# Alexander-H-Liu/End-to-end-ASR-Pytorch

Hardware: AMD Instinct MI355X
Metric: audio frames/sec training (LAS+CTC, LibriSpeech 80-mel) (higher is better)
Workload: dtype f32; 1 GPU; cfg3: {"B": 32, "T": 1600, "D": 80, "V": 5000, "L": 64}; global_batch=32, parallelism=dp1

## Files before the change

end-to-end-asr-pytorch_amd/csrc/speller.hip:

```cpp
#include "common.h"
#include "knobs.h"
#include <cstdlib>

namespace {

__device__ __forceinline__ float tanh_fast(float x) {
    const float e = __expf(2.f * x);
    return 1.f - __fdividef(2.f, e + 1.f);
}
__device__ __forceinline__ float sigmoid_fast(float x) { return __fdividef(1.f, 1.f + __expf(-x)); }

unsigned long long *g_sp_dbg = nullptr;
int g_sp_dbg_slots = 0;
inline unsigned long long *sp_slot(int step, int kid) {
    const long i = (long)step * 16 + kid;
    return (g_sp_dbg && i < g_sp_dbg_slots) ? g_sp_dbg + i * 16 : nullptr;
}
#define SP_STAMP(ph)                                                                                     \
    do {                                                                                                 \
        if (p.stamps && threadIdx.x == 0) {                                                              \
            if (blockIdx.x == 0 && blockIdx.y == 0) p.stamps[ph] = __builtin_readcyclecounter();         \
            else if (blockIdx.x == gridDim.x - 1 && blockIdx.y == gridDim.y - 1 && ((ph) == 0 || (ph) == 9)) \
                p.stamps[(ph) == 0 ? 12 : 13] = __builtin_readcyclecounter();                            \
        }                                                                                                \
// ... 33 lines not shown
};

template <int VEC>
__device__ __forceinline__ void load8(const float *row, int k, int klen, bool valid, float (&v)[8]) {
    if (VEC && valid && k + 8 <= klen) {
        const f32x4 a = *reinterpret_cast<const f32x4 *>(row + k);
        const f32x4 b = *reinterpret_cast<const f32x4 *>(row + k + 4);
        v[0] = a[0]; v[1] = a[1]; v[2] = a[2]; v[3] = a[3];
        v[4] = b[0]; v[5] = b[1]; v[6] = b[2]; v[7] = b[3];
        return;
    }
#pragma unroll
    for (int j = 0; j < 8; ++j) v[j] = (valid && k + j < klen) ? row[k + j] : 0.f;
}

template <int MT, int EPI, int VEC>
__global__ __launch_bounds__(SK_THREADS) void skinny_kernel(SkArgs p) {
    __shared__ float red[SK_WAVES][MT][4][64];
    const int tid = threadIdx.x, lane = tid & 63;
    const int wave = __builtin_amdgcn_readfirstlane(tid >> 6);
    const int slot = lane & 15, g = lane >> 4;
    SP_STAMP(0);
    int r;
    bool rvalid;
    if (EPI == EPI_LSTM_FWD) {
        const int u = blockIdx.x * 4 + (slot >> 2);
        r = (slot & 3) * p.H + u;
        rvalid = u < p.H;
    } else {
        r = blockIdx.x * 16 + slot;
        rvalid = r < p.R;
    }
    f32x4 acc[MT][2];
#pragma unroll
    for (int mt = 0; mt < MT; ++mt) acc[mt][0] = acc[mt][1] = f32x4{0.f, 0.f, 0.f, 0.f};

    float e_in[EPI == EPI_LSTM_BWD ? 36 : 13];
    const bool e_thr = tid < MT * 64;
    const int e_m = (tid >> 6) * 16 + (lane & 15);
    if (e_thr && e_m < p.M) {
        if (EPI == EPI_STORE || EPI == EPI_TANH_BIAS) {
#pragma unroll
            for (int q = 0; q < 4; ++q) {
                const int rr = blockIdx.x * 16 + (lane >> 4) * 4 + q;
                e_in[q] = (rr < p.R && p.bias) ? p.bias[rr] : 0.f;
            }
        } else if (EPI == EPI_LSTM_FWD) {
            const int u = blockIdx.x * 4 + (lane >> 4), H = p.H;
            if (u < H) {
#pragma unroll
                for (int q = 0; q < 4; ++q) {
                    const long col = (long)q * H + u;
                    e_in[q] = p.pre ? p.pre[(long)e_m * 4 * H + col] : 0.f;
                    e_in[4 + q] = p.b0 ? p.b0[col] : 0.f;
                    e_in[8 + q] = p.b1 ? p.b1[col] : 0.f;
                }
                e_in[12] = p.c_prev[(long)e_m * H + u];
            }
        } else {
            const int H = p.H;
#pragma unroll
            for (int q = 0; q < 4; ++q) {
                const int j = blockIdx.x * 16 + (lane >> 4) * 4 + q;
                if (j >= H) continue;
                const float *gr = p.dG + (long)e_m * 4 * H + j;
                e_in[q * 9 + 0] = p.add0 ? p.add0[(long)e_m * p.ld0 + j] : 0.f;
                e_in[q * 9 + 1] = p.add1 ? p.add1[(long)e_m * p.ld1 + j] : 0.f;
                e_in[q * 9 + 2] = gr[0];
                e_in[q * 9 + 3] = gr[H];
                e_in[q * 9 + 4] = gr[2 * (long)H];
                e_in[q * 9 + 5] = gr[3 * (long)H];
                e_in[q * 9 + 6] = p.bc_new[(long)e_m * H + j];
                e_in[q * 9 + 7] = p.dc_valid ? p.dc[(long)e_m * H + j] : 0.f;
                e_in[q * 9 + 8] = p.bc_prev[(long)e_m * H + j];
            }
        }
    }

// ... 18 lines not shown
        const unsigned long long wp0 = sg64(p.seg[0].w), wp1 = sg64(p.seg[1].w), wp2 = sg64(p.seg[2].w);
        const unsigned long long xp0 = sg64(p.seg[0].x), xp1 = sg64(p.seg[1].x), xp2 = sg64(p.seg[2].x);
        const unsigned wb0 = sg(p.seg[0].wbytes), wb1 = sg(has1 ? p.seg[1].wbytes : 0u), wb2 = sg(has2 ? p.seg[2].wbytes : 0u);
        const unsigned xb0 = sg(p.seg[0].xbytes), xb1 = sg(has1 ? p.seg[1].xbytes : 0u), xb2 = sg(has2 ? p.seg[2].xbytes : 0u);
        const unsigned ldw0 = sg((unsigned)p.seg[0].ldw * 4u), ldw1 = sg((unsigned)p.seg[1].ldw * 4u), ldw2 = sg((unsigned)p.seg[2].ldw * 4u);
        const unsigned ldx0 = sg((unsigned)p.seg[0].ldx * 4u), ldx1 = sg((unsigned)p.seg[1].ldx * 4u), ldx2 = sg((unsigned)p.seg[2].ldx * 4u);
        const unsigned kl0 = sg((unsigned)p.seg[0].klen * 4u), kl1 = sg(has1 ? (unsigned)p.seg[1].klen * 4u : 0u),
                       kl2 = sg(has2 ? (unsigned)p.seg[2].klen * 4u : 0u);
        const int Mrows = (int)sg((unsigned)p.M);
        unsigned wrow[2];
        bool wok[2];
#pragma unroll
        for (int h = 0; h < 2; ++h) {
            const int sl = lrow + 8 * h;
            if (EPI == EPI_LSTM_FWD) {
                const int u = blockIdx.x * 4 + (sl >> 2);
                wrow[h] = (unsigned)((sl & 3) * p.H + u);
                wok[h] = u < p.H;
            } else {
                wrow[h] = (unsigned)(blockIdx.x * 16 + sl);
                wok[h] = (int)wrow[h] < p.R;
            }
        }
#define SK_ISSUE(i_, gw_, gx_)                                                                          \
    do {                                                                                                \
        const int c_ = wave + (i_) * SK_WAVES;                \
        const bool s1_ = c_ >= n0, s2_ = c_ >= n0 + n1;                                                 \
        const int base_ = s2_ ? n0 + n1 : (s1_ ? n0 : 0);                                               \
        const __amdgpu_buffer_rsrc_t rw_ = __builtin_amdgcn_make_buffer_rsrc(                           \
            reinterpret_cast<void *>(s2_ ? wp2 : (s1_ ? wp1 : wp0)), 0, (int)(s2_ ? wb2 : (s1_ ? wb1 : wb0)), 0x00020000); \
        const __amdgpu_buffer_rsrc_t rx_ = __builtin_amdgcn_make_buffer_rsrc(                           \
            reinterpret_cast<void *>(s2_ ? xp2 : (s1_ ? xp1 : xp0)), 0, (int)(s2_ ? xb2 : (s1_ ? xb1 : xb0)), 0x00020000); \
        const unsigned ldw_ = s2_ ? ldw2 : (s1_ ? ldw1 : ldw0), ldx_ = s2_ ? ldx2 : (s1_ ? ldx1 : ldx0); \
        const unsigned kl_ = s2_ ? kl2 : (s1_ ? kl1 : kl0);                                             \
        const unsigned kb_ = (unsigned)(c_ - base_) * (SK_CH * 4u) + (unsigned)lk * 4u;                 \
// ... 27 lines not shown
        };
        auto mfmas = [&acc](const f32x4 (&fw)[2], const f32x4 (&fx)[MT][2]) __attribute__((always_inline)) {
#pragma unroll
            for (int hh = 0; hh < 2; ++hh)
#pragma unroll
                for (int j = 0; j < 4; ++j)
#pragma unroll
                    for (int mt = 0; mt < MT; ++mt)
                        acc[mt][j & 1] = __builtin_amdgcn_mfma_f32_16x16x4f32(fw[hh][j], fx[mt][hh][j], acc[mt][j & 1], 0, 0, 0);
        };
        if (mych > 0) {
            u32x4 gw[NB][2], gx[NB][NX];
            f32x4 fw[2][2], fx[2][MT][2];
#pragma unroll
            for (int j = 0; j < NB; ++j) SK_ISSUE(j, gw[j], gx[j]);
            SP_STAMP(1);
            stage(gw[0], gx[0], fw[0], fx[0]);
            SP_STAMP(2);
            SK_ISSUE(NB, gw[0], gx[0]);
#define SK_STEP(u)                                                                                      \
    if (i0 + (u) >= mych) break;                                                                        \
    stage(gw[((u) + 1) % NB], gx[((u) + 1) % NB], fw[((u) + 1) & 1], fx[((u) + 1) & 1]);                \
    SK_ISSUE(i0 + (u) + 1 + NB, gw[((u) + 1) % NB], gx[((u) + 1) % NB]);                                \
    __builtin_amdgcn_sched_barrier(0);                                                                  \
    mfmas(fw[(u) & 1], fx[(u) & 1]);                                                                    \
    __builtin_amdgcn_sched_barrier(0);
            for (int i0 = 0; i0 < mych; i0 += NB) {
                SK_STEP(0)
                SK_STEP(1)
                if (NB > 2) {
                    SK_STEP(2)
                    SK_STEP(3)
                }
// ... 22 lines not shown
#pragma unroll
                for (int mt = 0; mt < MT; ++mt)
                    acc[mt][j & 1] = __builtin_amdgcn_mfma_f32_16x16x4f32(w0[j], x0[mt][j], acc[mt][j & 1], 0, 0, 0);
#pragma unroll
            for (int j = 0; j < 8; ++j)
#pragma unroll
                for (int mt = 0; mt < MT; ++mt)
                    acc[mt][j & 1] = __builtin_amdgcn_mfma_f32_16x16x4f32(w1[j], x1[mt][j], acc[mt][j & 1], 0, 0, 0);
        }
    }
    }
#pragma unroll
    for (int mt = 0; mt < MT; ++mt)
#pragma unroll
        for (int v = 0; v < 4; ++v) red[wave][mt][v][lane] = acc[mt][0][v] + acc[mt][1][v];
    SP_STAMP(3);
    __syncthreads();
    SP_STAMP(4);
    if (tid >= MT * 64) return;
    const int mt = tid >> 6;
    float v[4];
#pragma unroll
    for (int q = 0; q < 4; ++q) {
        float s = 0.f;
#pragma unroll
        for (int w = 0; w < SK_WAVES; ++w) s += red[w][mt][q][lane];
        v[q] = s;
    }
    const int m = mt * 16 + (lane & 15);
    if (m >= p.M) return;
    if (EPI == EPI_STORE || EPI == EPI_TANH_BIAS) {
#pragma unroll
        for (int q = 0; q < 4; ++q) {
            const int rr = blockIdx.x * 16 + (lane >> 4) * 4 + q;
            if (rr < p.R) {
                float y = v[q] + e_in[q];
                if (EPI == EPI_TANH_BIAS) y = tanh_fast(y);
                p.out[(long)m * p.ldo + rr] = y;
            }
        }
    } else if (EPI == EPI_LSTM_FWD) {
        const int u = blockIdx.x * 4 + (lane >> 4);
        if (u >= p.H) return;
        const int H = p.H;
        float a[4];
#pragma unroll
        for (int q = 0; q < 4; ++q) {
            const long col = (long)q * H + u;
            (void)col;
            a[q] = v[q] + e_in[q] + e_in[4 + q] + e_in[8 + q];
        }
        float hn;
        if (p.gru) {
            const float gr_ = sigmoid_fast(a[0]), gz = sigmoid_fast(a[1]), gn = tanh_fast(a[2] + gr_ * a[3]);
            hn = (1.f - gz) * gn + gz * e_in[12];
            if (p.gates) {
                float *gr = p.gates + (long)m * 4 * H + u;
// ... 4 lines not shown
                        go = sigmoid_fast(a[3]);
            const float cn = gf * e_in[12] + gi * gg;
            hn = go * tanh_fast(cn);
            if (p.gates) {
                float *gr = p.gates + (long)m * 4 * H + u;
                gr[0] = gi; gr[H] = gf; gr[2 * (long)H] = gg; gr[3 * (long)H] = go;
            }
            p.c_new[(long)m * H + u] = cn;
        }
        p.h_new[(long)m * H + u] = hn;
        if (p.h_bm) p.h_bm[(long)m * p.h_bm_ld + u] = hn;
    } else {
        const int H = p.H;
#pragma unroll
        for (int q = 0; q < 4; ++q) {
            const int j = blockIdx.x * 16 + (lane >> 4) * 4 + q;
            if (j >= H) continue;
            float *gr = p.dG + (long)m * 4 * H + j;
            if (p.gru) {
                const float dh = v[q] + e_in[q * 9 + 0] + e_in[q * 9 + 1] + e_in[q * 9 + 7];
                const float r_ = e_in[q * 9 + 2], z_ = e_in[q * 9 + 3], n_ = e_in[q * 9 + 4], nh = e_in[q * 9 + 5];
                const float dnp = dh * (1.f - z_) * (1.f - n_ * n_);
                gr[0] = dnp * nh * r_ * (1.f - r_);
                gr[H] = dh * (e_in[q * 9 + 8] - n_) * z_ * (1.f - z_);
                gr[2 * (long)H] = dnp;
                gr[3 * (long)H] = dnp * r_;
                p.dc[(long)m * H + j] = dh * z_;
                continue;
            }
            const float dh = v[q] + e_in[q * 9 + 0] + e_in[q * 9 + 1];
            const float gi = e_in[q * 9 + 2], gf = e_in[q * 9 + 3], gg = e_in[q * 9 + 4], go = e_in[q * 9 + 5];
            const float tc = tanh_fast(e_in[q * 9 + 6]);
            const float dct = dh * go * (1.f - tc * tc) + e_in[q * 9 + 7];
            gr[0] = dct * gg * gi * (1.f - gi);
            gr[H] = dct * e_in[q * 9 + 8] * gf * (1.f - gf);
            gr[2 * (long)H] = dct * gi * (1.f - gg * gg);
            gr[3 * (long)H] = dh * tc * go * (1.f - go);
            p.dc[(long)m * H + j] = dct * gf;
        }
    }
    SP_STAMP(9);
}

inline bool al16(const void *q) { return (reinterpret_cast<uintptr_t>(q) & 15) == 0; }

template <int EPI>
int launch_skinny(const SkArgs &a, hipStream_t s) {
    if (a.M <= 0) return ASRK_OK;
    bool vec = true;
    for (int i = 0; i < a.nseg; ++i)
        vec = vec && al16(a.seg[i].x) && al16(a.seg[i].w) && a.seg[i].ldx % 4 == 0 && a.seg[i].ldw % 4 == 0 &&
              a.seg[i].klen % 4 == 0;
    const int blocks = (EPI == EPI_LSTM_FWD) ? asrk_div_up(a.H, 4) : asrk_div_up(a.R, 16);
    if (blocks <= 0) return ASRK_OK;
    for (int m0 = 0; m0 < a.M; m0 += 64) {
        SkArgs p = a;
        p.M = a.M - m0 < 64 ? a.M - m0 : 64;
        for (int i = 0; i < p.nseg; ++i) p.seg[i].x += (long)m0 * p.seg[i].ldx;
        bool small = true;
        const long wrows = (EPI == EPI_LSTM_FWD) ? 4L * p.H : (long)p.R;
        for (int i = 0; i < p.nseg; ++i) {
            const long wb = ((wrows - 1) * p.seg[i].ldw + p.seg[i].klen) * 4L;
            const long xb = ((long)(p.M - 1) * p.seg[i].ldx + p.seg[i].klen) * 4L;
            small = small && wb < (1L << 31) && xb < (1L << 31);
            p.seg[i].wbytes = (unsigned)wb;
            p.seg[i].xbytes = (unsigned)xb;
        }
        for (int i = p.nseg; i < 3; ++i) p.seg[i] = SkSeg{nullptr, nullptr, 0, 0, 0, 0u, 0u};
        if (p.out) p.out += (long)m0 * p.ldo;
        const long H4 = 4L * p.H, H1 = p.H;
        if (p.pre) p.pre += m0 * H4;
        if (p.c_prev) p.c_prev += m0 * H1;
        if (p.c_new) p.c_new += m0 * H1;
        if (p.h_new) p.h_new += m0 * H1;
        if (p.gates) p.gates += m0 * H4;
        if (p.h_bm) p.h_bm += (long)m0 * p.h_bm_ld;
        if (p.add0) p.add0 += (long)m0 * p.ld0;
        if (p.add1) p.add1 += (long)m0 * p.ld1;
        if (p.dG) p.dG += m0 * H4;
        if (p.bc_prev) p.bc_prev += m0 * H1;
        if (p.bc_new) p.bc_new += m0 * H1;
        if (p.dc) p.dc += m0 * H1;
        const int mt = p.M <= 16 ? 1 : (p.M <= 32 ? 2 : 4);
#define SK_LAUNCH_V(MT_, V_)                                                                        \
    do {                                                                                            \
        static AsrkLdsLatch latch_;                                                                 \
        const size_t lds = (size_t)SK_WAVES * (16 + MT_ * 16) * 36 * sizeof(float);                 \
        hipError_t e_ = asrk_max_lds_once(latch_, reinterpret_cast<const void *>(&skinny_kernel<MT_, EPI, V_>), (int)lds); \
        if (e_ != hipSuccess) return (int)e_;                                                       \
        hipLaunchKernelGGL((skinny_kernel<MT_, EPI, V_>), dim3(blocks), dim3(SK_THREADS), lds, s, p); \
    } while (0)
#define SK_LAUNCH(MT_)                                                                              \
    do {                                                                                            \
        if (vec && small) SK_LAUNCH_V(MT_, 2);                                                      \
        else hipLaunchKernelGGL((skinny_kernel<MT_, EPI, 0>), dim3(blocks), dim3(SK_THREADS), 0, s, p); \
    } while (0)
        if (mt == 1) SK_LAUNCH(1);
        else if (mt == 2) SK_LAUNCH(2);
        else SK_LAUNCH(4);
#undef SK_LAUNCH
#undef SK_LAUNCH_V
    }
// ... 876 lines not shown
#pragma unroll
        for (int w = 0; w < 8; ++w) acc += s_dq[w][a];
        p.dq_part[((long)r * TC + chunk) * A + a] = acc;
    }
}

struct CbArgs {
    const float *dconv, *prev, *Wc, *dq_part, *q;
    float *dprev, *dWc_part, *dq_pre;
    long prev_ld;
    int Te, K, ks, TC, A, nT, want_dprev;
    unsigned long long *stamps;
    int dq_only;
};

__global__ __launch_bounds__(256) void conv_bwd_kernel(CbArgs p) {
    extern __shared__ float sm[];
    const int b = blockIdx.x, y = p.dq_only ? p.nT + p.K : blockIdx.y, tid = threadIdx.x;
    const int Te = p.Te, K = p.K, ks = p.ks, KW = 2 * ks + 1;
    SP_STAMP(0);
    if (y < p.nT) {
        if (!p.want_dprev) return;
        const int s0 = y * 64, span = 64 + 2 * ks;
        float *sd = sm, *part = sm + K * span;
        float *s_w = part + 256;
        for (int i = tid; i < span * K; i += 256) {
            const int o = i / K, k = i - o * K;
            const int t = s0 + o - ks;
            sd[k * span + o] = (t >= 0 && t < Te) ? p.dconv[((long)b * Te + t) * K + k] : 0.f;
        }
        for (int i = tid; i < K * KW; i += 256) s_w[i] = p.Wc[i];
        __syncthreads();
        const int sl = tid & 63, w = __builtin_amdgcn_readfirstlane(tid >> 6);
        float acc = 0.f;
        for (int k = w; k < K; k += 4) {
            const float *wr = s_w + k * KW;
            const float *col = sd + k * span + sl + 2 * ks;
            for (int j = 0; j < KW; ++j) acc += col[-j] * wr[j];
        }
        part[w * 64 + sl] = acc;
        __syncthreads();
        if (tid < 64 && s0 + tid < Te)
            p.dprev[(long)b * Te + s0 + tid] = (part[tid] + part[64 + tid]) + (part[128 + tid] + part[192 + tid]);
        SP_STAMP(9);
    } else if (y < p.nT + K) {
        const int k = y - p.nT;
        float *s_dc = sm, *s_pv = sm + Te;
        float old[4];
#pragma unroll
        for (int r = 0; r < 4; ++r) {
            const int j = tid + 256 * r;
            old[r] = j < KW ? p.dWc_part[((long)b * K + k) * KW + j] : 0.f;
        }
        for (int t = tid; t < Te; t += 256) s_dc[t] = p.dconv[((long)b * Te + t) * K + k];
        for (int i = tid; i < Te + 2 * ks; i += 256) {
            const int t = i - ks;
            s_pv[i] = (t >= 0 && t < Te) ? p.prev[(long)b * p.prev_ld + t] : 0.f;
        }
        __syncthreads();
#pragma unroll
        for (int r = 0; r < 4; ++r) {
            const int j = tid + 256 * r;
            if (j < KW) {
                const float *pv = s_pv + j;
                float acc = 0.f;
                for (int t = 0; t < Te; ++t) acc += s_dc[t] * pv[t];
                p.dWc_part[((long)b * K + k) * KW + j] = old[r] + acc;
            }
        }
        for (int j = tid + 1024; j < KW; j += 256) {
            const float *pv = s_pv + j;
            float acc = 0.f;
            for (int t = 0; t < Te; ++t) acc += s_dc[t] * pv[t];
            p.dWc_part[((long)b * K + k) * KW + j] += acc;
        }
    } else {
        for (int a = tid; a < p.A; a += 256) {
            float acc = 0.f;
            for (int c = 0; c < p.TC; ++c) acc += p.dq_part[((long)b * p.TC + c) * p.A + a];
            const float qv = p.q[(long)b * p.A + a];
            p.dq_pre[(long)b * p.A + a] = acc * (1.f - qv * qv);
        }
        SP_STAMP(9);
    }
}

constexpr int DV_LC = 64;
__global__ __launch_bounds__(256) void dvalue_kernel(const float *__restrict__ attn, long attn_ld,
                                                     long attn_step, const float *__restrict__ dxh,
                                                     long step_ld, long row_ld, float *__restrict__ dvalue,
                                                     int L, int Te, int Dv) {
    extern __shared__ float s_at[];
    const int b = blockIdx.x, d = blockIdx.y * 256 + threadIdx.x;
    for (int l0 = 0; l0 < L; l0 += DV_LC) {
        const int nl = min(DV_LC, L - l0);
        __syncthreads();
        for (int i = threadIdx.x; i < nl * Te; i += 256) {
            const int l = i / Te, t = i - l * Te;
// ... 1 lines not shown
        }
        for (int i = nl * Te + threadIdx.x; i < DV_LC * Te; i += 256) s_at[i] = 0.f;
        __syncthreads();
        if (d < Dv) {
            float g[DV_LC];
#pragma unroll
            for (int l = 0; l < DV_LC; ++l)
                g[l] = l < nl ? dxh[(long)(l0 + l) * step_ld + (long)b * row_ld + d] : 0.f;
            float *out = dvalue + (long)b * Te * Dv + d;
            for (int t = 0; t < Te; ++t) {
                float acc = 0.f;
#pragma unroll
                for (int l = 0; l < DV_LC; ++l) acc += s_at[l * Te + t] * g[l];
                if (l0 == 0) out[(long)t * Dv] = acc;
                else out[(long)t * Dv] += acc;
            }
        }
    }
}

__global__ __launch_bounds__(256) void joint_score_kernel(const float *__restrict__ att,
                                                          const int64_t *__restrict__ cand,
                                                          const float *__restrict__ psi,
                                                          const float *__restrict__ prev_ctc,
                                                          const float *__restrict__ lm, float *__restrict__ out,
                                                          int V, int C, float wa, float w_ctc, float w_lm,
                                                          float logzero) {
    const int r = blockIdx.x;
    const float *a = att + (long)r * V;
    const float *l = lm ? lm + (long)r * V : nullptr;
// ... 132 lines not shown
inline bool upper_ok(const asrk_speller_t &d, bool fwd) {
    for (int l = 1; l < n_layers(d); ++l)
        if (!d.Wu_ih[l - 1] || !d.Wu_hh[l - 1] || !d.hu[l - 1] || !d.cu[l - 1] || !d.gu[l - 1] ||
            (fwd && (!d.bu_ih[l - 1] || !d.bu_hh[l - 1])))
            return false;
    return true;
}

template <typename T>
int set_lds(T kernel, size_t bytes) {
    ASRK_HIP(hipFuncSetAttribute(reinterpret_cast<const void *>(kernel),
                                 hipFuncAttributeMaxDynamicSharedMemorySize, (int)bytes));
    return ASRK_OK;
}

}

extern "C" void asrk_prof_launches_(int id, int64_t n);

extern "C" int asrk_transpose_ld_f32(const float *in, int64_t ldi, float *out, int64_t ldo, int rows,
                                     int cols, void *stream) {
    if (rows < 0 || cols < 0 || ldi < cols || ldo < rows) return ASRK_EINVAL;
    if (rows == 0 || cols == 0) return ASRK_OK;
    if (!in || !out) return ASRK_EINVAL;
    hipLaunchKernelGGL(transpose_ld_kernel, dim3(asrk_div_up(cols, 32), asrk_div_up(rows, 32)), dim3(256), 0,
                       (hipStream_t)stream, in, (long)ldi, out, (long)ldo, rows, cols);
    ASRK_LAUNCH_CHECK();
    return ASRK_OK;
}

extern "C" int asrk_speller_dvalue_f32(const float *attn, int64_t attn_ld, int64_t attn_step, const float *dxh,
                                       int64_t step_ld, int64_t row_ld, float *dvalue, int B, int L, int Te,
                                       int Dv, void *stream) {
    if (B < 0 || L <= 0 || Te <= 0 || Dv <= 0) return ASRK_EINVAL;
    if (B == 0) return ASRK_OK;
    if (!attn || !dxh || !dvalue) return ASRK_EINVAL;
    const size_t lds = (size_t)DV_LC * Te * sizeof(float);
    if (lds > LDS_BUDGET) return ASRK_ESHAPE;
    int rc = set_lds(dvalue_kernel, lds);
    if (rc) return rc;
    hipLaunchKernelGGL(dvalue_kernel, dim3(B, asrk_div_up(Dv, 256)), dim3(256), lds, (hipStream_t)stream, attn,
                       (long)attn_ld, (long)attn_step, dxh, (long)step_ld, (long)row_ld, dvalue, L, Te, Dv);
    ASRK_LAUNCH_CHECK();
    return ASRK_OK;
}

extern "C" void asrk_speller_set_debug_(void *buf, int slots) {
    g_sp_dbg = reinterpret_cast<unsigned long long *>(buf);
    g_sp_dbg_slots = slots;
}

// ... 280 lines not shown
        SkArgs a{};
        a.nseg = 1;
        a.seg[0] = SkSeg{g_of(*d, l) + (long)st * B * 4 * H, g->WuT[l - 1], 4L * H, 4L * H, 4 * H};
        a.M = B; a.R = 2 * H; a.H = H;
        a.out = g->dxu[l - 1] + (long)st * B * 2 * H; a.ldo = 2L * H;
        return launch_skinny<EPI_STORE>(a, s);
    };
    for (int l = top; l >= 0; --l) {
        rc = cell_bwd(l, L - 1, nullptr, nullptr, 0, -1);
        if (rc) return rc;
        if (l >= 1) {
            rc = upper_dx(l, L - 1);
            if (rc) return rc;
        }
    }
    for (int t = L - 1; t >= 0; --t) {
        float *dG_t = d->gates + (long)t * B * 4 * H;
        float *dxh_t = g->dxh + (long)t * B * XH;
        {
            SkArgs a{};
            a.nseg = 1;
            a.seg[0] = SkSeg{dG_t, g->WT, 4L * H, 4L * H, 4 * H};
            a.M = B; a.R = (int)XH; a.H = H;
            a.out = dxh_t; a.ldo = XH;
            a.stamps = sp_slot(t, 4);
            rc = launch_skinny<EPI_STORE>(a, s);
            if (rc) return rc;
        }
        const float *attn_t = d->attn + (long)t * d->attn_step;
        const float *dctx_rows = dxh_t;
        long dctx_ld = XH;
        if (NH > 1) {
            SkArgs a{};
            a.nseg = 1;
            a.seg[0] = SkSeg{dxh_t, g->WmT, XH, (long)Dv, Dv};
            a.M = B; a.R = NH * Dv; a.H = H;
            float *dctxh_t = g->dctxh + (long)t * BN * Dv;
            a.out = dctxh_t; a.ldo = (long)NH * Dv;
            rc = launch_skinny<EPI_STORE>(a, s);
            if (rc) return rc;
            dctx_rows = dctxh_t;
// ... 26 lines not shown
                     g->dq_part, g->dwe_part, g->dWp_part, g->dbe_part, d->attn_ld, Te, A, K, pl.tpb_b,
                     pl.KP, 1.f / d->temperature};
            a.stamps = sp_slot(t, 6);
            const dim3 grid(B, pl.tc_b);
            if (!pl.eb3_na) hipLaunchKernelGGL(energy_bwd_kernel2, grid, dim3(512), pl.lds_b, s, a);
            else if (pl.eb3_na == 2 && pl.eb3_km == 12) hipLaunchKernelGGL((energy_bwd_kernel3<2, 12>), grid, dim3(512), pl.lds_b3, s, a);
            else if (pl.eb3_na == 2) hipLaunchKernelGGL((energy_bwd_kernel3<2, 16>), grid, dim3(512), pl.lds_b3, s, a);
            else if (pl.eb3_km == 12) hipLaunchKernelGGL((energy_bwd_kernel3<5, 12>), grid, dim3(512), pl.lds_b3, s, a);
            else hipLaunchKernelGGL((energy_bwd_kernel3<5, 16>), grid, dim3(512), pl.lds_b3, s, a);
        }
        {
            const float *prev = t == 0 ? d->prev0 : d->attn + (long)(t - 1) * d->attn_step;
            CbArgs a{g->dconv, prev, d->Wc, g->dq_part, q_t, g->dprev, g->dWc_part, dq_pre_t,
                     t == 0 ? (long)Te : d->attn_ld, Te, K, d->ks, pl.tc_b, A, pl.nT, t > 0 ? 1 : 0};
            a.stamps = sp_slot(t, 7);
            hipLaunchKernelGGL(conv_bwd_kernel, dim3(B, pl.nT + K + 1), dim3(256), pl.lds_cb, s, a);
        }
        }
        if (t > 0) {
            for (int l = top; l >= 0; --l) {
                const float *hh = l == 0 ? dxh_t + Dv : g->dxu[l - 1] + (long)t * B * 2 * H + H;
                rc = cell_bwd(l, t - 1, dq_pre_t, hh, l == 0 ? XH : 2L * H, t);
                if (rc) return rc;
                if (l >= 1) {
                    rc = upper_dx(l, t - 1);
                    if (rc) return rc;
                }
            }
        }
        ASRK_LAUNCH_CHECK();
    }
    asrk_prof_end_(PROF_SPELLER, s);
    asrk_prof_launches_(PROF_SPELLER, (5L + 2 * (NL - 1) + (NH > 1)) * L - 1);
    return ASRK_OK;
}
```

end-to-end-asr-pytorch_amd/speller_ops.py:

```python
import ctypes
import os

import torch
from torch.autograd import Function

from . import _lib
from . import ops
from .ops import _L, _p, _stream, _f32c, _require_gpu, gemm, colsum, copy3d

c_int, c_i64, c_f32, c_vp = ctypes.c_int, ctypes.c_int64, ctypes.c_float, ctypes.c_void_p


class SpellerT(ctypes.Structure):
    _fields_ = ([(n, c_int) for n in ("B", "Te", "A", "Dv", "K", "ks", "H", "E", "L")]
                + [("temperature", c_f32), ("shared_kv", c_int)]
                + [(n, c_vp) for n in ("key", "value", "lens", "Wq", "bq", "Wc", "Wp", "we", "be", "W_ih",
                                       "W_hh", "b_ih", "b_hh", "eproj", "q", "conv", "attn")]
                + [("attn_ld", c_i64), ("attn_step", c_i64)]
                + [(n, c_vp) for n in ("ctx", "gates", "h", "c", "states", "e_scratch", "prev0", "row_mem")]
                + [("cell", c_int), ("nlayer", c_int)]
                + [(n, c_vp * 2) for n in ("Wu_ih", "Wu_hh", "bu_ih", "bu_hh", "hu", "cu", "gu")]
                + [("att_mode", c_int), ("nhead", c_int), ("Wm", c_vp), ("bm", c_vp), ("ctxh", c_vp)]
                + [("row_group", c_int)])


class SpellerBwdT(ctypes.Structure):
    _fields_ = ([(n, c_vp) for n in ("dstates", "dattn_seq", "WT", "WqT", "dkey", "dxh", "dq_pre", "dattn",
                                     "dprev", "dconv", "dq_part", "dwe_part", "dWp_part", "dbe_part",
                                     "dWc_part", "dc")]
                + [("tc", c_int)]
                + [(n, c_vp * 2) for n in ("WuT", "dxu", "dcu")]
                + [("WmT", c_vp), ("dctxh", c_vp)])


def _ptr(t):
    return t.data_ptr() if t is not None else None


MAX_LOOP_LAYERS = 3


def supported_train_loop(attention, decoder, training):
    if supported_loop(attention, decoder):
        return True
    if os.environ.get('ASRK_SPELLER', '1') == '0':
        return False
    att_ok = (attention.mode == 'loc' and attention.num_head == 1) or (attention.mode == 'dot' and attention.dim <= 512)
    dec_ok = decoder.layer == 1 or (decoder.enable_cell and decoder.layer <= MAX_LOOP_LAYERS
                                    and not (training and decoder.dropout > 0))
    return att_ok and dec_ok


def _set_slots(field, tensors):
    for i, t in enumerate(tensors):
# ... 81 lines not shown
        prev0 = uniform_attention(lens, Te) if not dot else torch.empty((1,), **f)
        d = SpellerT(B, Te, A, Dv, K, ks, H, E, L, float(temperature), 0,
                     _ptr(key), _ptr(value), _ptr(lens), _ptr(Wq), _ptr(bq), _ptr(Wc), _ptr(Wp), _ptr(we),
                     _ptr(be), _ptr(W_ih), _ptr(W_hh), _ptr(b_ih), _ptr(b_hh), _ptr(eproj), _ptr(tape['q']),
                     _ptr(tape['conv']), _ptr(att_seq), L * Te, Te, _ptr(tape['ctx']), _ptr(tape['gates']),
                     _ptr(tape['h']), _ptr(tape['c']) if cell == 0 else None, _ptr(states), _ptr(e_scratch),
                     _ptr(prev0))
        d.cell = int(cell)
        d.nlayer = NL
        d.att_mode, d.nhead = (1 if dot else 0), NH
        d.Wm, d.bm, d.ctxh = _ptr(Wm), _ptr(bm), (_ptr(tape['ctxh']) if NH > 1 else None)
        _set_slots(d.Wu_ih, upper[0::4]); _set_slots(d.Wu_hh, upper[1::4])
        _set_slots(d.bu_ih, upper[2::4]); _set_slots(d.bu_hh, upper[3::4])
        _set_slots(d.hu, [u['h'] for u in up_tape]); _set_slots(d.cu, [u['c'] for u in up_tape])
        _set_slots(d.gu, [u['g'] for u in up_tape])
        _lib.check(lib.asrk_speller_fwd_f32(ctypes.byref(d), _stream()), "speller_fwd")
        ctx.cell = int(cell)
        ctx.nlayer = NL
        ctx.nhead, ctx.dot = NH, dot
        ctx.merge = (Wm, tape['ctxh']) if NH > 1 else None
        ctx.dims = (B, Te, A, Dv, K, ks, H, E, L, float(temperature), teacher_emb.shape[1])
        ctx.save_for_backward(key, value, lens, emb_tm, Wq, bq, Wc, Wp, we, be, W_ih, W_hh, tape['q'],
                              tape['conv'], tape['ctx'], tape['gates'], tape['h'], tape['c'], att_seq, prev0,
                              *upper[0::4], *upper[1::4], *[u[n_] for n_ in ('h', 'c', 'g') for u in up_tape])
        ctx.weight_refs = tuple(t_ for t_ in (Wq, bq, Wc, Wp, we, be, W_ih, W_hh, b_ih, b_hh, Wm, bm) + tuple(upper)
                                if t_ is not None)
        ctx.consumed = False
        return states, att_seq

    @staticmethod
# ... 15 lines not shown
        dev = key.device
        f = dict(dtype=torch.float32, device=dev)
        In, XH, KW = E + Dv, Dv + H, 2 * ks + 1
        dstates = _f32c(dstates) if dstates is not None else ops.zeros((B, L, H), dev)
        datt = _f32c(datt_seq) if datt_seq is not None else None
        d = SpellerT(B, Te, A, Dv, K, ks, H, E, L, temperature, 0,
                     _ptr(key), _ptr(value), _ptr(lens), _ptr(Wq), _ptr(bq), _ptr(Wc), _ptr(Wp), _ptr(we),
                     _ptr(be), _ptr(W_ih), _ptr(W_hh), None, None, None, _ptr(q), _ptr(conv), _ptr(att_seq),
                     L * Te, Te, _ptr(ctx_all), _ptr(gates), _ptr(h), _ptr(c) if ctx.cell == 0 else None, None, None,
                     _ptr(prev0))
        d.cell = ctx.cell
        d.nlayer = NL
        d.att_mode, d.nhead = (1 if dot else 0), NH
        _set_slots(d.Wu_ih, Wu_ih); _set_slots(d.Wu_hh, Wu_hh)
        _set_slots(d.hu, hu); _set_slots(d.cu, cu); _set_slots(d.gu, gu)
        tc = c_int(0)
        _lib.check(lib.asrk_speller_plan(ctypes.byref(d), None, ctypes.byref(tc)), "speller_plan")
        tc = tc.value
        WT = torch.empty((XH, 4 * H), **f)
        transpose_into(W_ih[:, E:], In, 4 * H, Dv, WT, 4 * H)
        transpose_into(W_hh, H, 4 * H, H, WT[Dv:], 4 * H)
        WqT = torch.empty((NL * H, NA), **f)
        transpose_into(Wq, NL * H, NA, NL * H, WqT, NA)
        WmT = dctxh = None
        if NH > 1:
            Wm, ctxh_all = ctx.merge
            WmT = torch.empty((NH * Dv, Dv), **f)
            transpose_into(Wm, NH * Dv, Dv, NH * Dv, WmT, Dv)
            dctxh = torch.empty((L, B, NH * Dv), **f)
        WuT = []
# ... 243 lines not shown
```

include/asrk.h:

```cpp
#ifndef ASRK_H
#define ASRK_H

#include <stddef.h>
#include <stdint.h>

#ifdef __cplusplus
extern "C" {
#endif

#define ASRK_OK 0
#define ASRK_EINVAL (-1)
#define ASRK_ESHAPE (-2)
#define ASRK_EWORKSPACE (-3)
#define ASRK_EDEVICE (-4)
#define ASRK_ETIMEOUT (-5)

int asrk_version(void);
const char *asrk_strerror(int rc);
int asrk_init(int device);

void asrk_profile_enable(int on);
void asrk_profile_families(unsigned mask);
void asrk_profile_reset(void);
int asrk_profile_get(int id, double *total_ms, int64_t *launches);
// ... 173 lines not shown
    const float *Wq, *bq, *Wc, *Wp, *we, *be, *W_ih, *W_hh, *b_ih, *b_hh;
    const float *eproj;
    float *q, *conv, *attn;
    int64_t attn_ld, attn_step;
    float *ctx, *gates, *h, *c, *states, *e_scratch;
    const float *prev0;
    const int *row_mem;
    int cell;
    int nlayer;
    const float *Wu_ih[2], *Wu_hh[2], *bu_ih[2], *bu_hh[2];
    float *hu[2], *cu[2], *gu[2];
    int att_mode, nhead;
    const float *Wm, *bm;
    float *ctxh;
    int row_group;
} asrk_speller_t;
#define ASRK_SPELLER_MAX_LAYERS 3

typedef struct asrk_speller_bwd {
    const float *dstates, *dattn_seq, *WT, *WqT;
    float *dkey, *dxh, *dq_pre, *dattn, *dprev, *dconv, *dq_part, *dwe_part, *dWp_part, *dbe_part,
        *dWc_part, *dc;
    int tc;
    const float *WuT[2];
    float *dxu[2], *dcu[2];
    const float *WmT;
    float *dctxh;
} asrk_speller_bwd_t;

int asrk_speller_plan(const asrk_speller_t *dims, int *tc_fwd, int *tc_bwd);
// ... 172 lines not shown
```

Baseline: 533,700 frames/s.

## Co-schedule conv backward with next-step skinny GEMM and add MFMA dvalue kernel

```diff
diff --git a/end-to-end-asr-pytorch_amd/csrc/speller.hip b/end-to-end-asr-pytorch_amd/csrc/speller.hip
--- a/end-to-end-asr-pytorch_amd/csrc/speller.hip
+++ b/end-to-end-asr-pytorch_amd/csrc/speller.hip
@@ -71,21 +71,28 @@
     for (int j = 0; j < 8; ++j) v[j] = (valid && k + j < klen) ? row[k + j] : 0.f;
 }
 
+#define SK_STAMP(ph)                                                                                     \
+    do {                                                                                                 \
+        if (p.stamps && threadIdx.x == 0) {                                                              \
+            if (bid == 0) p.stamps[ph] = __builtin_readcyclecounter();                                   \
+            else if (bid == nblk - 1 && ((ph) == 0 || (ph) == 9))                                        \
+                p.stamps[(ph) == 0 ? 12 : 13] = __builtin_readcyclecounter();                            \
+        }                                                                                                \
+    } while (0)
 template <int MT, int EPI, int VEC>
-__global__ __launch_bounds__(SK_THREADS) void skinny_kernel(SkArgs p) {
-    __shared__ float red[SK_WAVES][MT][4][64];
+__device__ __forceinline__ void skinny_body(const SkArgs &p, const int bid, const int nblk, float (*red)[MT][4][64]) {
     const int tid = threadIdx.x, lane = tid & 63;
     const int wave = __builtin_amdgcn_readfirstlane(tid >> 6);
     const int slot = lane & 15, g = lane >> 4;
-    SP_STAMP(0);
+    SK_STAMP(0);
     int r;
     bool rvalid;
     if (EPI == EPI_LSTM_FWD) {
-        const int u = blockIdx.x * 4 + (slot >> 2);
+        const int u = bid * 4 + (slot >> 2);
         r = (slot & 3) * p.H + u;
         rvalid = u < p.H;
     } else {
-        r = blockIdx.x * 16 + slot;
+        r = bid * 16 + slot;
         rvalid = r < p.R;
     }
     f32x4 acc[MT][2];
@@ -99,11 +106,11 @@
         if (EPI == EPI_STORE || EPI == EPI_TANH_BIAS) {
 #pragma unroll
             for (int q = 0; q < 4; ++q) {
-                const int rr = blockIdx.x * 16 + (lane >> 4) * 4 + q;
+                const int rr = bid * 16 + (lane >> 4) * 4 + q;
                 e_in[q] = (rr < p.R && p.bias) ? p.bias[rr] : 0.f;
             }
         } else if (EPI == EPI_LSTM_FWD) {
-            const int u = blockIdx.x * 4 + (lane >> 4), H = p.H;
+            const int u = bid * 4 + (lane >> 4), H = p.H;
             if (u < H) {
 #pragma unroll
                 for (int q = 0; q < 4; ++q) {
@@ -118,7 +125,7 @@
             const int H = p.H;
 #pragma unroll
             for (int q = 0; q < 4; ++q) {
-                const int j = blockIdx.x * 16 + (lane >> 4) * 4 + q;
+                const int j = bid * 16 + (lane >> 4) * 4 + q;
                 if (j >= H) continue;
                 const float *gr = p.dG + (long)e_m * 4 * H + j;
                 e_in[q * 9 + 0] = p.add0 ? p.add0[(long)e_m * p.ld0 + j] : 0.f;
@@ -167,11 +174,11 @@
         for (int h = 0; h < 2; ++h) {
             const int sl = lrow + 8 * h;
             if (EPI == EPI_LSTM_FWD) {
-                const int u = blockIdx.x * 4 + (sl >> 2);
+                const int u = bid * 4 + (sl >> 2);
                 wrow[h] = (unsigned)((sl & 3) * p.H + u);
                 wok[h] = u < p.H;
             } else {
-                wrow[h] = (unsigned)(blockIdx.x * 16 + sl);
+                wrow[h] = (unsigned)(bid * 16 + sl);
                 wok[h] = (int)wrow[h] < p.R;
             }
         }
@@ -229,9 +236,9 @@
             f32x4 fw[2][2], fx[2][MT][2];
 #pragma unroll
             for (int j = 0; j < NB; ++j) SK_ISSUE(j, gw[j], gx[j]);
-            SP_STAMP(1);
+            SK_STAMP(1);
             stage(gw[0], gx[0], fw[0], fx[0]);
-            SP_STAMP(2);
+            SK_STAMP(2);
             SK_ISSUE(NB, gw[0], gx[0]);
 #define SK_STEP(u)                                                                                      \
     if (i0 + (u) >= mych) break;                                                                        \
@@ -284,9 +291,9 @@
     for (int mt = 0; mt < MT; ++mt)
 #pragma unroll
         for (int v = 0; v < 4; ++v) red[wave][mt][v][lane] = acc[mt][0][v] + acc[mt][1][v];
-    SP_STAMP(3);
+    SK_STAMP(3);
     __syncthreads();
-    SP_STAMP(4);
+    SK_STAMP(4);
     if (tid >= MT * 64) return;
     const int mt = tid >> 6;
     float v[4];
@@ -302,7 +309,7 @@
     if (EPI == EPI_STORE || EPI == EPI_TANH_BIAS) {
 #pragma unroll
         for (int q = 0; q < 4; ++q) {
-            const int rr = blockIdx.x * 16 + (lane >> 4) * 4 + q;
+            const int rr = bid * 16 + (lane >> 4) * 4 + q;
             if (rr < p.R) {
                 float y = v[q] + e_in[q];
                 if (EPI == EPI_TANH_BIAS) y = tanh_fast(y);
@@ -310,7 +317,7 @@
             }
         }
     } else if (EPI == EPI_LSTM_FWD) {
-        const int u = blockIdx.x * 4 + (lane >> 4);
+        const int u = bid * 4 + (lane >> 4);
         if (u >= p.H) return;
         const int H = p.H;
         float a[4];
@@ -345,7 +352,7 @@
         const int H = p.H;
 #pragma unroll
         for (int q = 0; q < 4; ++q) {
-            const int j = blockIdx.x * 16 + (lane >> 4) * 4 + q;
+            const int j = bid * 16 + (lane >> 4) * 4 + q;
             if (j >= H) continue;
             float *gr = p.dG + (long)m * 4 * H + j;
             if (p.gru) {
@@ -370,53 +377,76 @@
             p.dc[(long)m * H + j] = dct * gf;
         }
     }
-    SP_STAMP(9);
+    SK_STAMP(9);
+}
+#undef SK_STAMP
+
+template <int MT, int EPI, int VEC>
+__global__ __launch_bounds__(SK_THREADS) void skinny_kernel(SkArgs p) {
+    __shared__ float red[SK_WAVES][MT][4][64];
+    skinny_body<MT, EPI, VEC>(p, blockIdx.x, gridDim.x, red);
 }
 
 inline bool al16(const void *q) { return (reinterpret_cast<uintptr_t>(q) & 15) == 0; }
 
-template <int EPI>
-int launch_skinny(const SkArgs &a, hipStream_t s) {
-    if (a.M <= 0) return ASRK_OK;
+inline bool sk_vec(const SkArgs &a) {
     bool vec = true;
     for (int i = 0; i < a.nseg; ++i)
         vec = vec && al16(a.seg[i].x) && al16(a.seg[i].w) && a.seg[i].ldx % 4 == 0 && a.seg[i].ldw % 4 == 0 &&
               a.seg[i].klen % 4 == 0;
-    const int blocks = (EPI == EPI_LSTM_FWD) ? asrk_div_up(a.H, 4) : asrk_div_up(a.R, 16);
+    return vec;
+}
+template <int EPI>
+inline int sk_blocks(const SkArgs &a) { return (EPI == EPI_LSTM_FWD) ? asrk_div_up(a.H, 4) : asrk_div_up(a.R, 16); }
+constexpr size_t sk_lds(int mt) { return (size_t)SK_WAVES * (16 + mt * 16) * 36 * sizeof(float); }
+inline int sk_mt(int M) { return M <= 16 ? 1 : (M <= 32 ? 2 : 4); }
+
+template <int EPI>
+bool sk_pass(const SkArgs &a, int m0, SkArgs &p) {
+    p = a;
+    p.M = a.M - m0 < 64 ? a.M - m0 : 64;
+    for (int i = 0; i < p.nseg; ++i) p.seg[i].x += (long)m0 * p.seg[i].ldx;
+    bool small = true;
+    const long wrows = (EPI == EPI_LSTM_FWD) ? 4L * p.H : (long)p.R;
+    for (int i = 0; i < p.nseg; ++i) {
+        const long wb = ((wrows - 1) * p.seg[i].ldw + p.seg[i].klen) * 4L;
+        const long xb = ((long)(p.M - 1) * p.seg[i].ldx + p.seg[i].klen) * 4L;
+        small = small && wb < (1L << 31) && xb < (1L << 31);
+        p.seg[i].wbytes = (unsigned)wb;
+        p.seg[i].xbytes = (unsigned)xb;
+    }
+    for (int i = p.nseg; i < 3; ++i) p.seg[i] = SkSeg{nullptr, nullptr, 0, 0, 0, 0u, 0u};
+    if (p.out) p.out += (long)m0 * p.ldo;
+    const long H4 = 4L * p.H, H1 = p.H;
+    if (p.pre) p.pre += m0 * H4;
+    if (p.c_prev) p.c_prev += m0 * H1;
+    if (p.c_new) p.c_new += m0 * H1;
+    if (p.h_new) p.h_new += m0 * H1;
+    if (p.gates) p.gates += m0 * H4;
+    if (p.h_bm) p.h_bm += (long)m0 * p.h_bm_ld;
+    if (p.add0) p.add0 += (long)m0 * p.ld0;
+    if (p.add1) p.add1 += (long)m0 * p.ld1;
+    if (p.dG) p.dG += m0 * H4;
+    if (p.bc_prev) p.bc_prev += m0 * H1;
+    if (p.bc_new) p.bc_new += m0 * H1;
+    if (p.dc) p.dc += m0 * H1;
+    return small;
+}
+
+template <int EPI>
+int launch_skinny(const SkArgs &a, hipStream_t s) {
+    if (a.M <= 0) return ASRK_OK;
+    const bool vec = sk_vec(a);
+    const int blocks = sk_blocks<EPI>(a);
     if (blocks <= 0) return ASRK_OK;
     for (int m0 = 0; m0 < a.M; m0 += 64) {
-        SkArgs p = a;
-        p.M = a.M - m0 < 64 ? a.M - m0 : 64;
-        for (int i = 0; i < p.nseg; ++i) p.seg[i].x += (long)m0 * p.seg[i].ldx;
-        bool small = true;
-        const long wrows = (EPI == EPI_LSTM_FWD) ? 4L * p.H : (long)p.R;
-        for (int i = 0; i < p.nseg; ++i) {
-            const long wb = ((wrows - 1) * p.seg[i].ldw + p.seg[i].klen) * 4L;
-            const long xb = ((long)(p.M - 1) * p.seg[i].ldx + p.seg[i].klen) * 4L;
-            small = small && wb < (1L << 31) && xb < (1L << 31);
-            p.seg[i].wbytes = (unsigned)wb;
-            p.seg[i].xbytes = (unsigned)xb;
-        }
-        for (int i = p.nseg; i < 3; ++i) p.seg[i] = SkSeg{nullptr, nullptr, 0, 0, 0, 0u, 0u};
-        if (p.out) p.out += (long)m0 * p.ldo;
-        const long H4 = 4L * p.H, H1 = p.H;
-        if (p.pre) p.pre += m0 * H4;
-        if (p.c_prev) p.c_prev += m0 * H1;
-        if (p.c_new) p.c_new += m0 * H1;
-        if (p.h_new) p.h_new += m0 * H1;
-        if (p.gates) p.gates += m0 * H4;
-        if (p.h_bm) p.h_bm += (long)m0 * p.h_bm_ld;
-        if (p.add0) p.add0 += (long)m0 * p.ld0;
-        if (p.add1) p.add1 += (long)m0 * p.ld1;
-        if (p.dG) p.dG += m0 * H4;
-        if (p.bc_prev) p.bc_prev += m0 * H1;
-        if (p.bc_new) p.bc_new += m0 * H1;
-        if (p.dc) p.dc += m0 * H1;
-        const int mt = p.M <= 16 ? 1 : (p.M <= 32 ? 2 : 4);
+        SkArgs p;
+        const bool small = sk_pass<EPI>(a, m0, p);
+        const int mt = sk_mt(p.M);
 #define SK_LAUNCH_V(MT_, V_)                                                                        \
     do {                                                                                            \
         static AsrkLdsLatch latch_;                                                                 \
-        const size_t lds = (size_t)SK_WAVES * (16 + MT_ * 16) * 36 * sizeof(float);                 \
+        const size_t lds = sk_lds(MT_);                                                             \
         hipError_t e_ = asrk_max_lds_once(latch_, reinterpret_cast<const void *>(&skinny_kernel<MT_, EPI, V_>), (int)lds); \
         if (e_ != hipSuccess) return (int)e_;                                                       \
         hipLaunchKernelGGL((skinny_kernel<MT_, EPI, V_>), dim3(blocks), dim3(SK_THREADS), lds, s, p); \
@@ -1323,9 +1353,8 @@
     int dq_only;
 };
 
-__global__ __launch_bounds__(256) void conv_bwd_kernel(CbArgs p) {
-    extern __shared__ float sm[];
-    const int b = blockIdx.x, y = p.dq_only ? p.nT + p.K : blockIdx.y, tid = threadIdx.x;
+__device__ __forceinline__ void conv_bwd_body(const CbArgs &p, const int b, const int y, const int tid, float *sm,
+                                              const bool live) {
     const int Te = p.Te, K = p.K, ks = p.ks, KW = 2 * ks + 1;
     SP_STAMP(0);
     if (y < p.nT) {
@@ -1349,7 +1378,7 @@
         }
         part[w * 64 + sl] = acc;
         __syncthreads();
-        if (tid < 64 && s0 + tid < Te)
+        if (live && tid < 64 && s0 + tid < Te)
             p.dprev[(long)b * Te + s0 + tid] = (part[tid] + part[64 + tid]) + (part[128 + tid] + part[192 + tid]);
         SP_STAMP(9);
     } else if (y < p.nT + K) {
@@ -1367,6 +1396,7 @@
             s_pv[i] = (t >= 0 && t < Te) ? p.prev[(long)b * p.prev_ld + t] : 0.f;
         }
         __syncthreads();
+        if (!live) return;
 #pragma unroll
         for (int r = 0; r < 4; ++r) {
             const int j = tid + 256 * r;
@@ -1391,6 +1421,25 @@
             p.dq_pre[(long)b * p.A + a] = acc * (1.f - qv * qv);
         }
         SP_STAMP(9);
+    }
+}
+
+__global__ __launch_bounds__(256) void conv_bwd_kernel(CbArgs p) {
+    extern __shared__ float sm[];
+    conv_bwd_body(p, blockIdx.x, p.dq_only ? p.nT + p.K : blockIdx.y, threadIdx.x, sm, true);
+}
+
+template <int MT, int EPI, int VEC>
+__global__ __launch_bounds__(SK_THREADS) void skinny_conv_kernel(SkArgs a, CbArgs c, int nA, int B, int cb_floats) {
+    __shared__ float red[SK_WAVES][MT][4][64];
+    if ((int)blockIdx.x < nA) {
+        skinny_body<MT, EPI, VEC>(a, blockIdx.x, nA, red);
+    } else {
+        extern __shared__ float sm[];
+        const int i = blockIdx.x - nA, BH = (B + 1) >> 1;
+        const int half = __builtin_amdgcn_readfirstlane((int)threadIdx.x >> 8);
+        const int y = i / BH, b = (i - y * BH) * 2 + half;
+        conv_bwd_body(c, min(b, B - 1), y, threadIdx.x & 255, sm + half * cb_floats, b < B);
     }
 }
 
@@ -1422,6 +1471,67 @@
                 for (int l = 0; l < DV_LC; ++l) acc += s_at[l * Te + t] * g[l];
                 if (l0 == 0) out[(long)t * Dv] = acc;
                 else out[(long)t * Dv] += acc;
+            }
+        }
+    }
+}
+
+constexpr int DVM_DT = 4;
+__global__ __launch_bounds__(256) void dvalue_mfma_kernel(const float *__restrict__ attn, long attn_ld,
+                                                          long attn_step, const float *__restrict__ dxh,
+                                                          long step_ld, long row_ld, float *__restrict__ dvalue,
+                                                          int L, int Te, int Dv, int P) {
+    extern __shared__ float s_at[];
+    const int b = blockIdx.x, tid = threadIdx.x, lane = tid & 63;
+    const int wave = __builtin_amdgcn_readfirstlane(tid >> 6);
+    const int i16 = lane & 15, g = lane >> 4;
+    const int dbase = blockIdx.y * 256 + wave * (16 * DVM_DT);
+    const int TeP = (Te + 15) & ~15;
+    for (int l0 = 0; l0 < L; l0 += DV_LC) {
+        const int nl = min(DV_LC, L - l0);
+        __syncthreads();
+        for (int l = wave; l < DV_LC; l += 4) {
+            const float *ar = attn + (long)b * attn_ld + (long)(l0 + min(l, nl - 1)) * attn_step;
+            for (int t = lane; t < P; t += 64) s_at[l * P + t] = (l < nl && t < Te) ? ar[t] : 0.f;
+        }
+        __syncthreads();
+        if (dbase >= Dv) continue;
+        const int nks = (nl + 3) >> 2;
+        float a[DVM_DT][DV_LC / 4];
+#pragma unroll
+        for (int ks = 0; ks < DV_LC / 4; ++ks) {
+            const int l = 4 * ks + g;
+            const float *dr = dxh + (long)(l0 + min(l, nl - 1)) * step_ld + (long)b * row_ld;
+#pragma unroll
+            for (int dt = 0; dt < DVM_DT; ++dt) {
+                const int d = dbase + 16 * dt + i16;
+                a[dt][ks] = (l < nl && d < Dv) ? dr[min(d, Dv - 1)] : 0.f;
+            }
+        }
+        for (int t0 = 0; t0 < TeP; t0 += 16) {
+            f32x4 acc[DVM_DT];
+#pragma unroll
+            for (int dt = 0; dt < DVM_DT; ++dt) acc[dt] = f32x4{0.f, 0.f, 0.f, 0.f};
+#pragma unroll
+            for (int ks = 0; ks < DV_LC / 4; ++ks) {
+                if (ks < nks) {
+                    const float bv = s_at[(4 * ks + g) * P + t0 + i16];
+#pragma unroll
+                    for (int dt = 0; dt < DVM_DT; ++dt)
+                        acc[dt] = __builtin_amdgcn_mfma_f32_16x16x4f32(a[dt][ks], bv, acc[dt], 0, 0, 0);
+                }
+            }
+            const int t = t0 + i16;
+            if (t < Te) {
+#pragma unroll
+                for (int dt = 0; dt < DVM_DT; ++dt) {
+                    const int d = dbase + 16 * dt + 4 * g;
+                    if (d < Dv) {
+                        f32x4 *o = reinterpret_cast<f32x4 *>(dvalue + ((long)b * Te + t) * Dv + d);
+                        if (l0 == 0) *o = acc[dt];
+                        else *o = *o + acc[dt];
+                    }
+                }
             }
         }
     }
@@ -1584,6 +1694,36 @@
     return ASRK_OK;
 }
 
+template <int EPI>
+int launch_skinny_conv(const SkArgs &a, const CbArgs &c, int B, size_t lds_cb, unsigned &attr_done, hipStream_t s) {
+    const int nA = sk_blocks<EPI>(a), nC = ((B + 1) / 2) * (c.nT + c.K);
+    const int mt = sk_mt(a.M);
+    SkArgs pa;
+    const bool vec = sk_vec(a) && sk_pass<EPI>(a, 0, pa);
+    const int cb_floats = (int)((lds_cb + 15) / 16) * 4;
+    const size_t lds = std::max(vec ? sk_lds(mt) : (size_t)0, 2 * (size_t)cb_floats * sizeof(float));
+    if (a.M <= 0 || a.M > 64 || nA <= 0 || lds + (size_t)SK_WAVES * mt * 4 * 64 * sizeof(float) > 160 * 1024) {
+        hipLaunchKernelGGL(conv_bwd_kernel, dim3(B, c.nT + c.K), dim3(256), lds_cb, s, c);
+        return launch_skinny<EPI>(a, s);
+    }
+    sk_pass<EPI>(a, 0, pa);
+#define CC_LAUNCH(MT_, V_)                                                                          \
+    do {                                                                                            \
+        if (!(attr_done & (1u << (V_ ? 1 : 0)))) {                                                  \
+            int rc_ = set_lds(skinny_conv_kernel<MT_, EPI, V_>, lds);                               \
+            if (rc_) return rc_;                                                                    \
+            attr_done |= 1u << (V_ ? 1 : 0);                                                        \
+        }                                                                                           \
+        hipLaunchKernelGGL((skinny_conv_kernel<MT_, EPI, V_>), dim3(nA + nC), dim3(SK_THREADS), lds, s, pa, c, nA, B, cb_floats); \
+    } while (0)
+    if (mt == 1) { if (vec) CC_LAUNCH(1, 2); else CC_LAUNCH(1, 0); }
+    else if (mt == 2) { if (vec) CC_LAUNCH(2, 2); else CC_LAUNCH(2, 0); }
+    else { if (vec) CC_LAUNCH(4, 2); else CC_LAUNCH(4, 0); }
+#undef CC_LAUNCH
+    ASRK_LAUNCH_CHECK();
+    return ASRK_OK;
+}
+
 }
 
 extern "C" void asrk_prof_launches_(int id, int64_t n);
@@ -1605,6 +1745,18 @@
     if (B < 0 || L <= 0 || Te <= 0 || Dv <= 0) return ASRK_EINVAL;
     if (B == 0) return ASRK_OK;
     if (!attn || !dxh || !dvalue) return ASRK_EINVAL;
+    if (Dv % 4 == 0 && al16(dvalue)) {
+        const int TeP = (Te + 15) & ~15, P = TeP % 32 == 16 ? TeP : TeP + 16;
+        const size_t lds_m = (size_t)DV_LC * P * sizeof(float);
+        if (lds_m <= LDS_BUDGET) {
+            int rc = set_lds(dvalue_mfma_kernel, lds_m);
+            if (rc) return rc;
+            hipLaunchKernelGGL(dvalue_mfma_kernel, dim3(B, asrk_div_up(Dv, 256)), dim3(256), lds_m, (hipStream_t)stream,
+                               attn, (long)attn_ld, (long)attn_step, dxh, (long)step_ld, (long)row_ld, dvalue, L, Te, Dv, P);
+            ASRK_LAUNCH_CHECK();
+            return ASRK_OK;
+        }
+    }
     const size_t lds = (size_t)DV_LC * Te * sizeof(float);
     if (lds > LDS_BUDGET) return ASRK_ESHAPE;
     int rc = set_lds(dvalue_kernel, lds);
@@ -1915,6 +2067,9 @@
             if (rc) return rc;
         }
     }
+    CbArgs pending_conv{};
+    bool have_pending = false;
+    unsigned b2_attr = 0;
     for (int t = L - 1; t >= 0; --t) {
         float *dG_t = d->gates + (long)t * B * 4 * H;
         float *dxh_t = g->dxh + (long)t * B * XH;
@@ -1925,7 +2080,12 @@
             a.M = B; a.R = (int)XH; a.H = H;
             a.out = dxh_t; a.ldo = XH;
             a.stamps = sp_slot(t, 4);
-            rc = launch_skinny<EPI_STORE>(a, s);
+            if (have_pending) {
+                rc = launch_skinny_conv<EPI_STORE>(a, pending_conv, B, pl.lds_cb, b2_attr, s);
+                have_pending = false;
+            } else {
+                rc = launch_skinny<EPI_STORE>(a, s);
+            }
             if (rc) return rc;
         }
         const float *attn_t = d->attn + (long)t * d->attn_step;
@@ -1982,7 +2142,15 @@
             CbArgs a{g->dconv, prev, d->Wc, g->dq_part, q_t, g->dprev, g->dWc_part, dq_pre_t,
                      t == 0 ? (long)Te : d->attn_ld, Te, K, d->ks, pl.tc_b, A, pl.nT, t > 0 ? 1 : 0};
             a.stamps = sp_slot(t, 7);
-            hipLaunchKernelGGL(conv_bwd_kernel, dim3(B, pl.nT + K + 1), dim3(256), pl.lds_cb, s, a);
+            if (d->chain && t > 0) {
+                pending_conv = a;
+                pending_conv.stamps = nullptr;
+                have_pending = true;
+                a.dq_only = 1;
+                hipLaunchKernelGGL(conv_bwd_kernel, dim3(B, 1), dim3(256), pl.lds_cb, s, a);
+            } else {
+                hipLaunchKernelGGL(conv_bwd_kernel, dim3(B, pl.nT + K + 1), dim3(256), pl.lds_cb, s, a);
+            }
         }
         }
         if (t > 0) {
@@ -1999,6 +2167,6 @@
         ASRK_LAUNCH_CHECK();
     }
     asrk_prof_end_(PROF_SPELLER, s);
-    asrk_prof_launches_(PROF_SPELLER, (5L + 2 * (NL - 1) + (NH > 1)) * L - 1);
+    asrk_prof_launches_(PROF_SPELLER, (5L + 2 * (NL - 1) + (NH > 1)) * L - 1 + ((d->chain && loc) ? L - 1 : 0));
     return ASRK_OK;
 }
diff --git a/end-to-end-asr-pytorch_amd/speller_ops.py b/end-to-end-asr-pytorch_amd/speller_ops.py
--- a/end-to-end-asr-pytorch_amd/speller_ops.py
+++ b/end-to-end-asr-pytorch_amd/speller_ops.py
@@ -21,7 +21,7 @@
                 + [("cell", c_int), ("nlayer", c_int)]
                 + [(n, c_vp * 2) for n in ("Wu_ih", "Wu_hh", "bu_ih", "bu_hh", "hu", "cu", "gu")]
                 + [("att_mode", c_int), ("nhead", c_int), ("Wm", c_vp), ("bm", c_vp), ("ctxh", c_vp)]
-                + [("row_group", c_int)])
+                + [("row_group", c_int), ("chain", c_int)])
 
 
 class SpellerBwdT(ctypes.Structure):
@@ -38,6 +38,7 @@
 
 
 MAX_LOOP_LAYERS = 3
+CHAIN = int(os.environ.get('ASRK_SPELLER_CHAIN', '1'))
 
 
 def supported_train_loop(attention, decoder, training):
@@ -149,6 +150,7 @@
         _set_slots(d.bu_ih, upper[2::4]); _set_slots(d.bu_hh, upper[3::4])
         _set_slots(d.hu, [u['h'] for u in up_tape]); _set_slots(d.cu, [u['c'] for u in up_tape])
         _set_slots(d.gu, [u['g'] for u in up_tape])
+        ctx.chain = int(CHAIN)
         _lib.check(lib.asrk_speller_fwd_f32(ctypes.byref(d), _stream()), "speller_fwd")
         ctx.cell = int(cell)
         ctx.nlayer = NL
@@ -194,6 +196,7 @@
         d.att_mode, d.nhead = (1 if dot else 0), NH
         _set_slots(d.Wu_ih, Wu_ih); _set_slots(d.Wu_hh, Wu_hh)
         _set_slots(d.hu, hu); _set_slots(d.cu, cu); _set_slots(d.gu, gu)
+        d.chain = ctx.chain
         tc = c_int(0)
         _lib.check(lib.asrk_speller_plan(ctypes.byref(d), None, ctypes.byref(tc)), "speller_plan")
         tc = tc.value
diff --git a/include/asrk.h b/include/asrk.h
--- a/include/asrk.h
+++ b/include/asrk.h
@@ -211,6 +211,7 @@
     const float *Wm, *bm;
     float *ctxh;
     int row_group;
+    int chain;
 } asrk_speller_t;
 #define ASRK_SPELLER_MAX_LAYERS 3
 
```

Result: no change. 537,400 frames/s, median of 6 (+0.7%).
